# digitalcytometry/cytospace

Hardware: AMD Instinct MI355X
Metric: cell-to-spot assignments/sec on NxN synthetic cost; bit-exact vs lapjv (higher is better)
Workload: dtype f32

## Files before the change

cytospace_amd/_lib.py:

```python
import ctypes
import os

_HERE = os.path.dirname(os.path.abspath(__file__))
LIB_PATH = os.environ.get("CYTOHIP_LIB") or os.path.join(_HERE, "libcytohip.so")
_lib = None

CYTO_OK = 0
CYTO_ERR_NONFINITE = 2
_EXC = {1: ValueError, 2: ValueError, 3: MemoryError, 7: ValueError, 8: ValueError}
CYTO_ERR_PEER = 9
CYTO_ERR_UNSUPPORTED = 7
CYTO_DTYPE_F32, CYTO_DTYPE_F64, CYTO_DTYPE_U16, CYTO_DTYPE_U8, CYTO_DTYPE_I32, CYTO_DTYPE_I64 = range(6)
CYTO_MTX_ERR_FRACTION, CYTO_MTX_ERR_NONFINITE, CYTO_MTX_ERR_MAGNITUDE, CYTO_MTX_ERR_SQUARE, CYTO_MTX_ERR_IO = range(2, 7)


class CytoHipError(RuntimeError):
    pass


class LapInfo(ctypes.Structure):
    _fields_ = [("ms_colred", ctypes.c_double), ("ms_cache", ctypes.c_double), ("ms_chain", ctypes.c_double),
                ("ms_total", ctypes.c_double)] + \
        [(k, ctypes.c_int64) for k in (
            "scans_colred", "scans_redtransfer", "scans_arr", "scans_aug_init", "scans_aug_relax",
# ... 55 lines not shown
def lib():
    global _lib
    if _lib is None:
        if not os.path.exists(LIB_PATH):
            raise CytoHipError(
                f"{LIB_PATH} not found: build it with `python -m cytospace_amd.build` "
                "(hipcc --offload-arch=gfx950). There is no CPU fallback.")
        L = ctypes.CDLL(LIB_PATH)
        L.cyto_strerror.restype = ctypes.c_char_p
        L.cyto_strerror.argtypes = [ctypes.c_int]
        L.cyto_last_hip_error.restype = ctypes.c_char_p
        L.cyto_version.restype = ctypes.c_char_p
        vp, i32, i64 = ctypes.c_void_p, ctypes.c_int, ctypes.c_int64
        L.cyto_device_count.argtypes = [ctypes.POINTER(ctypes.c_int)]
        L.cyto_device_name.argtypes = [i32, ctypes.c_char_p, ctypes.c_size_t]
        L.cyto_malloc.argtypes = [ctypes.POINTER(vp), ctypes.c_size_t, i32]
        L.cyto_free.argtypes = [vp, i32]
        L.cyto_memcpy_h2d.argtypes = [vp, vp, ctypes.c_size_t, i32]
        L.cyto_memcpy_d2h.argtypes = [vp, vp, ctypes.c_size_t, i32]
        L.cyto_device_synchronize.argtypes = [i32]
        for name in ("cyto_lap_f32", "cyto_lap_f64"):
            getattr(L, name).argtypes = [i32, vp, i64, i32, vp, vp, vp, vp, ctypes.POINTER(ctypes.c_double),
                                         ctypes.POINTER(LapInfo), i32, vp]
        for name in ("cyto_lap_f32_opts", "cyto_lap_f64_opts"):
            getattr(L, name).argtypes = [i32, vp, i64, i32, vp, vp, vp, vp, ctypes.POINTER(ctypes.c_double),
                                         ctypes.POINTER(LapInfo), i32, vp, ctypes.POINTER(LapOpts)]
            getattr(L, name).restype = ctypes.c_int
        L.cyto_lap_f32_rowmap.argtypes = [i32, vp, i64, i32, i32, vp, vp, vp, vp, vp, ctypes.POINTER(ctypes.c_double),
                                          ctypes.POINTER(LapInfo), i32, vp, ctypes.POINTER(LapOpts)]
        L.cyto_lap_f32_rowmap.restype = ctypes.c_int
        if hasattr(L, "cyto_wide_embedded_solves"):
            L.cyto_wide_embedded_solves.argtypes = []
            L.cyto_wide_embedded_solves.restype = ctypes.c_longlong
        L.cyto_trim_device_cache.argtypes = [i32]
        L.cyto_trim_device_cache.restype = ctypes.c_int
        dp = ctypes.POINTER(ctypes.c_double)
        L.cyto_lap_f32_from_f64.argtypes = [i32, vp, i64, vp, vp, vp, vp, ctypes.POINTER(ctypes.c_double),
                                            ctypes.POINTER(LapInfo), i32, vp]
        L.cyto_normalize_data.argtypes = [i32, i32, vp, i64, i32, vp, i64, i32]
        L.cyto_standardize.argtypes = [i32, i32, vp, i64, i32, i32, i32, vp, i64, i32, i32, vp]
        L.cyto_cost_pearson.argtypes = [i32, i32, i32, vp, i64, vp, i64, vp, vp, i64, dp, i32, vp]
        L.cyto_transform.argtypes = [i32, i32, i32, vp, i64, i32, i32, i32, vp, i64, i32, i32, vp]
        L.cyto_cost_metric.argtypes = [i32, i32, i32, i32, vp, i64, vp, i64, vp, vp, i64, dp, i32, vp]
        L.cyto_assign_metric.argtypes = [i32, i32, i32, i32, vp, vp, vp, i32, vp, dp, ctypes.POINTER(AssignInfo), i32]
        L.cyto_assign_metric_ex.argtypes = [i32, i32, ctypes.POINTER(Matrix), i32, ctypes.POINTER(Matrix), i32, vp, i32, vp, dp,
                                            ctypes.POINTER(AssignInfo), i32]
        L.cyto_assign_metric_ex.restype = ctypes.c_int
        L.cyto_ctx_create.argtypes = [i32, i32, i32, i32, vp, vp, i32, i32, ctypes.POINTER(vp)]
        L.cyto_ctx_assign_chunk.argtypes = [vp, vp, i32, vp, i32, vp, vp, dp, ctypes.POINTER(AssignInfo)]
        L.cyto_ctx_destroy.argtypes = [vp]
        L.cyto_assign_metric_typed.argtypes = [i32, i32, i32, i32, vp, vp, i32, vp, i32, vp, dp, ctypes.POINTER(AssignInfo), i32]
        L.cyto_ctx_create_typed.argtypes = [i32, i32, i32, i32, vp, vp, i32, i32, i32, ctypes.POINTER(vp)]
        L.cyto_ctx_destroy.restype = None
        L.cyto_ctx_create_shared.argtypes = [i32, i32, i32, i32, vp, vp, i32, i32, vp, i32, i32, i32, ctypes.POINTER(vp), dp]
        L.cyto_ctx_create_shared.restype = ctypes.c_int
        L.cyto_ctx_create_ex.argtypes = [i32, i32, ctypes.POINTER(Matrix), i32, ctypes.POINTER(Matrix), i32, i32, vp, i32, i32, i32,
                                         ctypes.POINTER(vp), dp]
        L.cyto_ctx_create_ex.restype = ctypes.c_int
        L.cyto_csc_to_dense_f32.argtypes = [i32, i32, i64, vp, vp, vp, vp, i64, i32, vp]
        L.cyto_csc_to_dense_f32.restype = ctypes.c_int
        L.cyto_ctx_assign_chunks.argtypes = [vp, i32, ctypes.POINTER(Chunk), i32]
        L.cyto_ctx_assign_chunks.restype = ctypes.c_int
        L.cyto_memcpy_d2d.argtypes = [vp, vp, ctypes.c_size_t, i32]
        L.cyto_memcpy_d2d.restype = ctypes.c_int
        L.cyto_assign_pearson.argtypes = [i32, i32, i32, vp, vp, vp, i32, vp, dp, ctypes.POINTER(AssignInfo), i32]
        L.cyto_lap_batch_f32.argtypes = [i32, vp, vp, vp, i32, vp, vp, vp, vp, vp, vp, vp, i32, i32]
# ... 33 lines not shown
            getattr(L, name).restype = ctypes.c_int
        sz = [ctypes.c_size_t() for _ in range(4)]
        L.cyto_abi_sizes.argtypes = [ctypes.POINTER(ctypes.c_size_t)] * 4
        L.cyto_abi_sizes(*[ctypes.byref(x) for x in sz])
        mine = [ctypes.sizeof(t) for t in (LapInfo, LapOpts, AssignInfo, Chunk)]
        if [x.value for x in sz] != mine:
            raise CytoHipError(f"{LIB_PATH} was built from another include/cytohip.h: struct sizes {[x.value for x in sz]} != {mine} "
                               "(rebuild: python -m cytospace_amd.build --force)")
        for name in ("cyto_normalize_data", "cyto_standardize", "cyto_cost_pearson", "cyto_assign_pearson",
                     "cyto_lap_batch_f32", "cyto_lap_batch_f32_opts", "cyto_comm_unique_id", "cyto_comm_init", "cyto_comm_bcast_f32",
                     "cyto_comm_destroy"):
            getattr(L, name).restype = ctypes.c_int
        for name in ("cyto_device_count", "cyto_device_name", "cyto_malloc", "cyto_free", "cyto_memcpy_h2d",
                     "cyto_memcpy_d2h", "cyto_device_synchronize", "cyto_lap_f32", "cyto_lap_f64"):
            getattr(L, name).restype = ctypes.c_int
        _lib = L
    return _lib


def check(status):
    if status == CYTO_OK:
        return
    L = lib()
    msg = L.cyto_strerror(status).decode()
    if status == 5:
        msg += ": " + L.cyto_last_hip_error().decode()
    raise _EXC.get(status, CytoHipError)(f"cytohip status {status}: {msg}")


def wide_embedded_solves():
    return int(lib().cyto_wide_embedded_solves())


def device_count():
    n = ctypes.c_int(0)
    st = lib().cyto_device_count(ctypes.byref(n))
    return n.value if st == CYTO_OK else 0


class DeviceBuffer:

    def __init__(self, nbytes, device_id=0):
        self.device_id = device_id
        self.nbytes = int(nbytes)
        p = ctypes.c_void_p()
        check(lib().cyto_malloc(ctypes.byref(p), self.nbytes, device_id))
        self.ptr = p.value

    @classmethod
    def from_numpy(cls, arr, device_id=0):
        import numpy as np
        arr = np.ascontiguousarray(arr)
        buf = cls(arr.nbytes, device_id)
        check(lib().cyto_memcpy_h2d(buf.ptr, arr.ctypes.data, arr.nbytes, device_id))
        return buf

    def clone(self):
        out = DeviceBuffer(self.nbytes, self.device_id)
        check(lib().cyto_memcpy_d2d(out.ptr, self.ptr, self.nbytes, self.device_id))
        return out

    def to_numpy(self, shape, dtype):
        import numpy as np
        out = np.empty(shape, dtype)
        assert out.nbytes <= self.nbytes
        check(lib().cyto_memcpy_d2h(out.ctypes.data, self.ptr, out.nbytes, self.device_id))
# ... 78 lines not shown
```

cytospace_amd/csrc/lap_wide.hip:

```cpp
#include "lap_dev.h"
#include "lap_wide.h"
#include <algorithm>
#include <atomic>
#include <chrono>
#include <mutex>
#include <thread>
#include <vector>

namespace cyto {

#define WIDE_FIELDS(P, S)                                                                                                  \
    S(int, n) S(int64_t, ld) P(const float, cost) P(const int32_t, rowmap) P(float, v) P(float, u) P(float, cassign)          \
    P(unsigned long long, label) P(unsigned long long, bid) P(int32_t, rowsol) P(int32_t, colsol) P(int32_t, matches)          \
    P(int32_t, freerows) P(int32_t, act0) P(int32_t, act1) P(int32_t, touched) P(int32_t, slot_j) P(float, slot_p)            \
    P(float, slot_c) P(uint32_t, cache_col) P(float, cache_val) P(char, misc) S(long long, max_rounds)                     \
    P(const int32_t, same_prev) P(int32_t, seg_sync) S(int, aug_seg) S(int, aug_waste) S(int, arr_waste) S(int, seg_quorum)   \
    P(char, sc) S(int, par_groups) P(char, par) P(char, scx) P(float, cache_red) P(const int32_t, inv_off) P(const unsigned long long, inv_ent)
#define WIDE_F_PTR(T, name) T *name;
#define WIDE_F_VAL(T, name) T name;
struct WideArgs { WIDE_FIELDS(WIDE_F_PTR, WIDE_F_VAL) };

constexpr size_t WIDE_SC_BYTES = 2048;

namespace {

constexpr int WT = 1024;
constexpr int WNW = WT / 64;
constexpr int RTB = 256;

template <typename T> __device__ __forceinline__ T ld_sc1(const T *p) { return __hip_atomic_load(p, __ATOMIC_RELAXED, __HIP_MEMORY_SCOPE_AGENT); }
template <typename T> __device__ __forceinline__ void st_sc1(T *p, T x) { __hip_atomic_store(p, x, __ATOMIC_RELAXED, __HIP_MEMORY_SCOPE_AGENT); }
__device__ __forceinline__ int64_t wrow_off(const int32_t *__restrict__ rowmap, int i, int64_t ld) {
    return (int64_t)(rowmap ? rowmap[i] : i) * ld;
}
#define WIDE_F_GPTR(T, name) __attribute__((address_space(1))) T *name;
#define WIDE_F_COPY_PTR(T, name) a.name = (T *)g.name;
#define WIDE_F_COPY_VAL(T, name) a.name = g.name;
// ... 989 lines not shown
        h->started = 1; h->round = round; h->bids = bids; h->retired = s.retired; h->dense = s.dense; h->cnt[cur] = paused ? na : 0;
        h->cnt[cur ^ 1] = 0; h->free_cr = free_cr; h->done = paused ? 0 : 1; h->launches += 1; h->list_rounds = n_list;
#ifndef CYTO_WIDE_PROF
        tmr[WT_ARR_LAUNCHES] = h->launches;
#endif
        if (a.seg_sync) a.seg_sync[1 + blockIdx.x] = (paused ? 1 : 0) | ((!paused && s.dense <= n / 64) ? 2 : 0);
    }
}

struct ClaimCtl { int changed, blocked, rounds, pad_; };
__device__ __forceinline__ int *cl_claim(const WideArgs &a) { return reinterpret_cast<int *>(a.scx); }
__device__ __forceinline__ unsigned long long *cl_mask(const WideArgs &a) { return reinterpret_cast<unsigned long long *>(a.scx + sc_np(a.n) * 8); }
__device__ __forceinline__ int2 *cl_state(const WideArgs &a) { return reinterpret_cast<int2 *>(a.scx + sc_np(a.n) * 16); }
__device__ __forceinline__ ClaimCtl *cl_ctl(const WideArgs &a) { return reinterpret_cast<ClaimCtl *>(a.scx + sc_np(a.n) * 24); }
__device__ __forceinline__ int *cl_rem(const WideArgs &a) { return reinterpret_cast<int *>(a.scx + sc_np(a.n) * 32); }
constexpr int AP = 2;

size_t wide_aug_lds_bytes(int n, bool vlds, bool clds) {
    const size_t nblk = ((size_t)n + 63) / 64, nw32 = ((size_t)n + 31) / 32, npad = ((size_t)n + 3) & ~(size_t)3;
    return ((nblk * 8 + 3 * nw32 * 4 + npad * ((vlds ? 4 : 0) + (clds ? 2 : 0)) + 15) / 16) * 16;
}
bool wide_aug_vlds(int n) { return n <= 65534 && wide_aug_lds_bytes(n, true, true) + 4096 <= (size_t)LDS_DYNAMIC_MAX; }
bool wide_aug_clds(int n) { return n <= 65534 && wide_aug_lds_bytes(n, false, true) + 4096 <= (size_t)LDS_DYNAMIC_MAX; }

struct AugShared {
    unsigned long long T;
    int ntouch, any[3], npk[3], fail, anydense, rootdense, doroot, f, err;
    int waste, stop;
    int nhop;
    int conflict;
    int scans;
    int st_row[64], st_col[64];
    float st_val[64];
};
static_assert(WNW * 2 <= 32, "the queue of a round's full-row relaxations: two halves of the 64-entry staging arrays");

struct ParCtl {
    unsigned int bar_arrive, bar_gen;
    int P[2], nplog[2], nolog[2];
    int err, pad_;
    long long c_relax, c_hops, c_proc, c_dense, c_rounds, c_verify, c_batches, c_discarded;
};
static_assert(sizeof(ParCtl) <= 256, "control block");
constexpr int PAR_GMAX = 64;
static size_t wide_par_state_bytes(int n, int G) {
    const size_t np = ((size_t)n + 63) & ~(size_t)63;
    return 256 + (size_t)G * np * 8 + (size_t)G * np * 4 + (size_t)G * np * 8 + np * 4 + np * 8 + np * 8;
}
__device__ __forceinline__ void par_barrier(ParCtl *c, int G, unsigned &gen) {
    __syncthreads();
    if (threadIdx.x == 0) {
        __builtin_amdgcn_fence(__ATOMIC_RELEASE, "agent");
        asm volatile("s_waitcnt vmcnt(0)" ::: "memory");
        const unsigned arrived = atomicAdd(&c->bar_arrive, 1u) + 1u;
        if (arrived == (gen + 1u) * (unsigned)G) st_sc1(&c->bar_gen, gen + 1u);
        else {
            long long spins = 0;
            while (ld_sc1(&c->bar_gen) <= gen) {
                __builtin_amdgcn_s_sleep(2);
                if (++spins > (1ll << 26)) { atomicExch(&c->err, 2); break; }
            }
        }
        __builtin_amdgcn_fence(__ATOMIC_ACQUIRE, "agent");
    }
    gen++;
    __syncthreads();
}

#ifndef CYTO_COOP_MIN_N
#define CYTO_COOP_MIN_N 16384
#endif
constexpr int COOP_MIN_N = CYTO_COOP_MIN_N;
template <bool VLDS>
__device__ __forceinline__ void coop_dense_rows(AugShared *sp, int nd, const float *__restrict__ cost, const int32_t *__restrict__ rowmap, int64_t ld,
                                             int n, int w, int lane, unsigned long long *lbl, int32_t *tch, uint32_t *dirty,
                                             unsigned long long *bmin, const uint32_t *asg, const float *s_v, const float *v) {
// ... 114 lines not shown
    auto is_asg = [&](int c) -> bool { return (asg[c >> 5] >> (c & 31)) & 1u; };

    long long c_relax = 0, c_hops = 0, c_rounds = 0, c_proc = 0, c_trivial = 0, c_dense = 0, c_verify = 0;
    long long t_rounds = 0, t_verify = 0, t_finish = 0, t_triv = 0, t_mark = wall_clock64();

#define AUG_LAP(acc) { const long long now_ = wall_clock64(); acc += now_ - t_mark; t_mark = now_; }

    auto offer = [&](int col, unsigned long long lv, int row) -> unsigned long long {
        return atomicMin(lbl + col, lkey(lv, (uint32_t)row));
    };
    auto after_offer = [&](int col, unsigned long long lv, int row, unsigned long long old) {
        const unsigned long long key = lkey(lv, (uint32_t)row);
        if (key < old) {
            if (old == ~0ull) tch[atomicAdd(&s.ntouch, 1)] = col;
            if (lv_of(old) > lv) {
                const unsigned long long ck = lkey(lv, (uint32_t)col);
                if (is_asg(col)) { atomicOr(&dirty[col >> 5], 1u << (col & 31)); atomicMin(&bmin[col >> 6], ck); }
                else atomicMin(&s.T, ck);
            }
        }
    };
    auto relax_to = [&](int col, unsigned long long lv, int row) { after_offer(col, lv, row, offer(col, lv, row)); };

    int f = f0;
    int ph = 0;
    int rb[AP];
#pragma unroll
    for (int q = 0; q < AP; q++) rb[q] = -1;
    int seg_done = 0;
    int wact = 4;
    bool announced = false;
    int fbase = 0, batchno = 1, perr = 0;
    long long c_batches = 0, c_discarded = 0;
    for (;;) {
        if (!PAR && w == 0) {
            auto flush_one_edge = [&](int cnt) {
                if (lane < cnt) {
                    const int r = s.st_row[lane], cc = s.st_col[lane];
                    a.rowsol[r] = cc; a.colsol[cc] = r; a.cassign[cc] = s.st_val[lane];
                }
            };
            const int *remp = (a.same_prev && a.scx) ? cl_rem(a) : nullptr;
            int nst = 0;
            int p0, l0, r0, p1, l1, r1, p2, l2, r2, p3, l3v, r3v;
            uint32_t col0, col1, col2; float val0, val1, val2, vv0, vv1;
            auto start = [&](int ff) {
                auto len_of = [&](int pp) -> int { return pp < numfree ? (remp ? uni(remp[pp]) : 1) : 1; };
                auto row_at = [&](int pp) -> int { return pp < numfree ? uni(a.freerows[pp]) : -1; };
                p0 = ff; l0 = len_of(p0); r0 = row_at(p0);
                p1 = p0 + l0; l1 = len_of(p1); r1 = row_at(p1);
                p2 = p1 + l1; l2 = len_of(p2); r2 = row_at(p2);
                p3 = p2 + l2; l3v = p3 < numfree ? (remp ? remp[p3] : 1) : 1; r3v = p3 < numfree ? a.freerows[p3] : -1;
                col0 = COLSENT; col1 = COLSENT; col2 = COLSENT; val0 = 0.0f; val1 = 0.0f; val2 = 0.0f;
                if (r0 >= 0) { col0 = a.cache_col[(int64_t)r0 * KC + lane]; val0 = a.cache_val[(int64_t)r0 * KC + lane]; }
                if (r1 >= 0) { col1 = a.cache_col[(int64_t)r1 * KC + lane]; val1 = a.cache_val[(int64_t)r1 * KC + lane]; }
                if (r2 >= 0) { col2 = a.cache_col[(int64_t)r2 * KC + lane]; val2 = a.cache_val[(int64_t)r2 * KC + lane]; }
                vv0 = (r0 >= 0 && lane < KCU && col0 != COLSENT) ? getv((int)col0) : 0.0f;
                vv1 = (r1 >= 0 && lane < KCU && col1 != COLSENT) ? getv((int)col1) : 0.0f;
            };
            start(f);
            while (f < numfree) {
                const int fr = r0, L = l0 < 1 ? 1 : l0;
                const uint32_t col = col0;
                const float val = val0, vv = vv0;
                const int n_p3 = p3, n_l3 = uni(l3v), n_r3 = uni(r3v);
                p0 = p1; l0 = l1; r0 = r1; col0 = col1; val0 = val1; vv0 = vv1;
// ... 19 lines not shown
                    s.st_row[nst + rank] = fr + rank; s.st_col[nst + rank] = (int)col; s.st_val[nst + rank] = val;
                    if (CLDS) s_cs[col] = (uint16_t)(fr + rank);
                    atomicOr(&asg[col >> 5], 1u << (col & 31));
                }
                c_trivial += m; c_hops += m;
                f += m;
                nst += m;
                if (nst == 64) { flush_one_edge(nst); nst = 0; }
                if (m != L && f < numfree) start(f);
            }
            flush_one_edge(nst);
            if (lane == 0) {
                s.f = f;
                if (seg_done > 0 && f < numfree) {
                    bool stop = a.aug_seg > 0 && seg_done >= a.aug_seg;
                    if (a.aug_seg == 0) {
                        if (s.waste >= a.aug_waste) { stop = true; if (!announced && a.seg_sync) atomicAdd(a.seg_sync, 1); announced = true; }
                        else if (a.seg_sync && a.seg_quorum > 0 && ld_sc1(a.seg_sync) >= a.seg_quorum) stop = true;
                    }
                    if (stop) s.stop = 1;
                }
            }
        }
        __syncthreads();
        AUG_LAP(t_triv)
        if (PAR) {
            if (fbase >= numfree || perr) break;
            f = fbase + g;
        } else {
            f = uni(s.f);
            if (f >= numfree || uni(s.stop)) break;
        }
        const bool active = !PAR || f < numfree;
        seg_done++;
        const int fr = a.freerows[active ? f : 0];
        const float *__restrict__ frow = a.cost + wrow_off(a.rowmap, fr, a.ld);
        const float ftau = a.cache_val[(int64_t)fr * KC + KCU];

        if (active) {
        if (w == 0) {
            const uint32_t col = a.cache_col[(int64_t)fr * KC + lane];
            const float val = a.cache_val[(int64_t)fr * KC + lane];
            if (EMB) {
                const float red = ld_sc1(a.cache_red + (int64_t)fr * KC + lane);
                if (lane < KCU && col != COLSENT) relax_to((int)col, (unsigned long long)f2ord(red) << 12, fr);
            } else if (lane < KCU && col != COLSENT) relax_to((int)col, (unsigned long long)f2ord(val - getv((int)col)) << 12, fr);
        }
        __syncthreads();

        for (;;) {
            int nd = 0;
            for (;;) {
                const unsigned long long Tlv = uni(lv_of(s.T));
                const int W = wact;
                if (w >= W && rb[0] < 0 && rb[1] < 0) {
                    __syncthreads();
                    const int any0 = uni(s.any[ph]), npd0 = uni(s.npk[ph]), np0 = npd0 & 0xFFFF;
                    ph = (ph + 1) % 3;
                    c_rounds++;
                    wact = np0 > 6 ? WNW : 4;
                    nd = npd0 >> 16;
                    if (!any0 || nd) break;
                    continue;
                }
                unsigned long long mk = ~0ull;
                if (w < W) for (int b = w + W * lane; b < nblk; b += W * 64) mk = umin64(mk, bmin[b]);
                bool pk[AP]; int pj[AP], oi[AP];
                unsigned long long lab[AP];
                float ca[AP], vp[AP], val[AP];
                uint32_t col[AP];
                {
                    uint32_t dk = lv_of(mk) < Tlv ? (uint32_t)(mk >> 32) : 0xFFFFFFFFu;
#pragma unroll
                    for (int q = 0; q < AP; q++) {
                        const uint32_t m = wave_min_u32(dk);
                        pk[q] = m != 0xFFFFFFFFu;
                        const int l = pk[q] ? __ffsll((unsigned long long)__ballot(dk == m)) - 1 : 0;
                        pj[q] = (int)(rdlane((uint32_t)mk, l) & 0xFFFFFu);
                        if (lane == l) dk = 0xFFFFFFFFu;
                    }
                }
#pragma unroll
                for (int q = 0; q < AP; q++) {
                    if (pk[q] && lane == 0) { atomicAnd(&dirty[pj[q] >> 5], ~(1u << (pj[q] & 31))); bmin[pj[q] >> 6] = ~0ull; }
                }
                if (lane == 0 && (pk[0] || pk[1] || rb[0] >= 0 || rb[1] >= 0)) { s.any[ph] = 1; if (pk[0]) atomicAdd(&s.npk[ph], (int)pk[0] + (int)pk[1]); }
                asm volatile("s_waitcnt lgkmcnt(0)" ::: "memory");
                int pjx[AP];
                unsigned long long lab_r[AP];
                float ca_r[AP], vp_r[AP];
                int oi_r[AP];
#pragma unroll
                for (int q = 0; q < AP; q++) {
                    pjx[q] = pk[q] ? pj[q] : 0;
                    lab_r[q] = ld_sc1(lbl + pjx[q]); ca_r[q] = ld_sc1(a.cassign + pjx[q]);
                }
                bool db[AP]; unsigned long long lbr[AP];
#pragma unroll
                for (int q = 0; q < AP; q++) {
                    const int c = (rb[q] < 0 ? 0 : rb[q]) * 64 + lane;
                    db[q] = rb[q] >= 0 && c < n && ((dirty[c >> 5] >> (c & 31)) & 1u);
                    lbr[q] = ld_sc1(lbl + (db[q] ? c : pjx[q]));
                }
#pragma unroll
                for (int q = 0; q < AP; q++) { vp_r[q] = getv(pjx[q]); oi_r[q] = getcs(pjx[q]); }
#pragma unroll
                for (int q = 0; q < AP; q++) {
                    oi[q] = uni(oi_r[q]);
                    const int oix = oi[q] < 0 ? 0 : oi[q];
                    col[q] = a.cache_col[(int64_t)oix * KC + lane];
                    val[q] = EMB ? ld_sc1(a.cache_red + (int64_t)oix * KC + lane) : a.cache_val[(int64_t)oix * KC + lane];
                }
#pragma unroll
                for (int q = 0; q < AP; q++) {
                    lab[q] = pk[q] ? uni(lab_r[q]) : ~0ull; ca[q] = uni(ca_r[q]); vp[q] = uni(vp_r[q]);
                    if (!pk[q]) { col[q] = COLSENT; oi[q] = 0; }
                }
                unsigned long long old[AP], co[AP];
                bool off[AP], dn[AP];
                float vc[AP];
#pragma unroll
                for (int q = 0; q < AP; q++) {
                    const bool valid = lane < KCU && col[q] != COLSENT;
                    vc[q] = EMB ? 0.0f : getv(valid ? (int)col[q] : pjx[q]);
                }
#pragma unroll
                for (int q = 0; q < AP; q++) {
                    off[q] = false; dn[q] = false; old[q] = 0; co[q] = 0;
                    const uint32_t dord = (uint32_t)(lab[q] >> 32), kq = (uint32_t)(lab[q] >> 20) & LKMAX;
                    if (pk[q] && lv_of(lab[q]) < Tlv) {
                        c_proc++;
                        if ((dense[oi[q] >> 5] >> (oi[q] & 31)) & 1u) { dn[q] = true; continue; }
                        const float h = (ca[q] - vp[q]) - ord2f(dord);
                        const unsigned long long lv = edge_lv(f2ord(EMB ? val[q] - h : (val[q] - vc[q]) - h), dord, kq);
                        off[q] = lane < KCU && col[q] != COLSENT && (int)col[q] != pj[q] && lv <= Tlv;
                        co[q] = lv;
                    }
                }
                {
                    static_assert(AP == 2, "two offers per wave and round");
                    const uint64_t m0 = __ballot(off[0]), m1 = __ballot(off[1]);
                    if (m0 | m1) {
                        unsigned long long *p0 = lbl + (off[0] ? (int)col[0] : 0), *p1 = lbl + (off[1] ? (int)col[1] : 0);
                        const unsigned long long k0 = lkey(co[0], (uint32_t)oi[0]), k1 = lkey(co[1], (uint32_t)oi[1]);
                        unsigned long long r0, r1;
                        uint64_t sv;
                        asm volatile("s_mov_b64 %[sv], exec\n\t"
                                     "s_and_b64 exec, %[sv], %[m0]\n\t"
                                     "global_atomic_umin_x2 %[r0], %[a0], %[d0], off sc0\n\t"
                                     "s_and_b64 exec, %[sv], %[m1]\n\t"
// ... 17 lines not shown
                    const uint32_t dord = (uint32_t)(lab[q] >> 32), kq = (uint32_t)(lab[q] >> 20) & LKMAX;
                    const float h = (ca[q] - vp[q]) - ord2f(dord);
                    if (n >= COOP_MIN_N) {
                        if (lane == 0) {
                            const int e = atomicAdd(&s.npk[ph], 1 << 16) >> 16;
                            s.st_row[e] = oi[q]; s.st_row[32 + e] = pj[q]; s.st_col[e] = (int)dord; s.st_col[32 + e] = (int)kq; s.st_val[e] = h;
                        }
                    } else {
                        const float *__restrict__ row = a.cost + wrow_off(a.rowmap, oi[q], a.ld);
                        const int pjq = pj[q], oiq = oi[q];
                        wave_row_sweep(row, n, lane, [&](int c, float x) {
                            const unsigned long long lv = edge_lv(f2ord((x - getv(c)) - h), dord, kq);
                            if (c != pjq && lv <= lv_of(s.T) && (lkey(lv, (uint32_t)oiq) < ld_sc1(lbl + c))) relax_to(c, lv, oiq);
                        });
                    }
                    c_dense++;
                    if (lane == 0) atomicAdd(&s.waste, 1);
                }
#pragma unroll
                for (int q = 0; q < AP; q++) {
                    if (rb[q] >= 0) {
                        const int c = rb[q] * 64 + lane;
                        const uint32_t dk = db[q] ? (uint32_t)(lbr[q] >> 32) : 0xFFFFFFFFu;
                        const uint32_t m = wave_min_u32(dk);
                        if (m != 0xFFFFFFFFu) {
                            const int l = __ffsll((unsigned long long)__ballot(dk == m)) - 1;
                            if (lane == 0) atomicMin(&bmin[rb[q]], ((unsigned long long)m << 32) | (uint32_t)(c - lane + l));
                        }
                    }
                    rb[q] = pk[q] ? (pj[q] >> 6) : -1;
                }
                __syncthreads();
                const int any = uni(s.any[ph]), npd = uni(s.npk[ph]), np = npd & 0xFFFF;
                if (tid == 0) { s.any[(ph + 2) % 3] = 0; s.npk[(ph + 2) % 3] = 0; }
                ph = (ph + 1) % 3;
                c_rounds++;
                wact = np > 6 ? WNW : 4;
                nd = npd >> 16;
                if (!any || nd) break;
            }
            if (nd) {
                coop_dense_rows<VLDS>(&s, nd, a.cost, a.rowmap, a.ld, n, w, lane, lbl, tch, dirty, bmin, asg, s_v, a.v);
                continue;
            }
            AUG_LAP(t_rounds)
            const unsigned long long Tk = s.T;
            const uint32_t Dord = (uint32_t)(Tk >> 32);
            const float D = Tk == ~0ull ? INFINITY : ord2f(Dord);
            const int nt = s.ntouch;
            for (int q = tid; q < nt; q += WT) {
                const int k = ld_sc1(tch + q);
                const unsigned long long lbk = ld_sc1(lbl + k);
                const uint32_t dord = (uint32_t)(lbk >> 32);
                if (lv_of(lbk) < lv_of(Tk) && is_asg(k)) {
                    const int i = getcs(k);
                    if (!((dense[i >> 5] >> (i & 31)) & 1u)) {
                        const float h = (ld_sc1(a.cassign + k) - getv(k)) - ord2f(dord);
                        const float bound = a.cache_val[(int64_t)i * KC + KCU] - h;
                        if (!(bound > D)) {
                            atomicOr(&dense[i >> 5], 1u << (i & 31));
                            atomicOr(&dirty[k >> 5], 1u << (k & 31));
                            atomicMin(&bmin[k >> 6], lkey(lv_of(lbk), (uint32_t)k));
                            atomicAdd(&s.fail, 1);
                        }
                    }
                }
            }
            if (tid == 0 && !s.rootdense && !(ftau > D)) { s.rootdense = 1; s.doroot = 1; atomicAdd(&s.fail, 1); }
            c_verify++;
            __syncthreads();
            const int fail = s.fail;
            if (s.doroot)
                for (int c = tid; c < n; c += WT) {
                    const unsigned long long lv = (unsigned long long)f2ord(frow[c] - getv(c)) << 12;
                    if (lv <= lv_of(s.T) && (lkey(lv, (uint32_t)fr) < ld_sc1(lbl + c))) relax_to(c, lv, fr);
                }
            __syncthreads();
            if (tid == 0) { if (fail) s.anydense = 1; s.fail = 0; s.doroot = 0; }
            __syncthreads();
            AUG_LAP(t_verify)
            if (!fail) break;
        }

        }

        const unsigned long long Tk = active ? s.T : ~0ull;
        if (!PAR && Tk == ~0ull) { if (tid == 0) s.err = 1; __syncthreads(); break; }
        const uint32_t Dord = (uint32_t)(Tk >> 32);
        const float D = ord2f(Dord);
        const int sink = (int)lid_of(Tk);
        const int nt = active ? s.ntouch : 0;
        bool commit = true;
        int Pb = G;
        const int par = batchno & 1;
        if (PAR) {
            const bool have = Tk != ~0ull;
            if (active && !have && tid == 0) atomicExch(&pc->err, 1);
            const uint32_t key = ((uint32_t)batchno << 8) | (uint32_t)(255 - g);
            if (have) {
                for (int q = tid; q < nt; q += WT) {
                    const int k = ld_sc1(tch + q);
                    if (lv_of(ld_sc1(lbl + k)) < lv_of(Tk) && is_asg(k)) atomicMax(claim + k, key);
                }
                if (tid == 0) atomicMax(claim + sink, key);
            }
            if (tid == 0) s.conflict = 0;
            par_barrier(pc, G, pgen);
            if (have) {
                int c = 0;
                for (int q = tid; q < nt; q += WT) {
                    const int k = ld_sc1(tch + q);
                    if (lv_of(ld_sc1(lbl + k)) < lv_of(Tk) && is_asg(k) && ld_sc1(claim + k) != key) c = 1;
                }
                if (tid == 0 && ld_sc1(claim + sink) != key) c = 1;
                if (c) s.conflict = 1;
            }
            __syncthreads();
            if (tid == 0 && active && (s.conflict || !have)) atomicMin(&pc->P[par], g);
            par_barrier(pc, G, pgen);
            Pb = uni(ld_sc1(&pc->P[par]));
            Pb = Pb < G ? Pb : G;
            if (g == 0 && tid == 0) { st_sc1(&pc->P[par ^ 1], PAR_GMAX + 1); st_sc1(&pc->nplog[par ^ 1], 0); st_sc1(&pc->nolog[par ^ 1], 0); }
            commit = active && have && g < Pb;
            if (active && !commit) c_discarded++;
        }
        if (commit) {
            int myscans = 0;
            for (int q = tid; q < nt; q += WT) {
                const int k = ld_sc1(tch + q);
                const uint32_t dord = (uint32_t)(ld_sc1(lbl + k) >> 32);
                if (dord < Dord && is_asg(k)) {
                    const float vk = getv(k);
                    const float nv = (vk + ord2f(dord)) - D;
                    if (nv < vk) {
                        a.v[k] = nv; if (VLDS) s_v[k] = nv;
                        if (PAR) { const int e = atomicAdd(&pc->nplog[par], 1); plog_col[e] = k; plog_val[e] = nv; }
                    }
                    myscans++;
                }
            }
            if (myscans) atomicAdd(&s.scans, myscans);
            if (tid == 0) {
                int j = sink, nh = 0;
                for (;;) {
                    const int i = (int)lid_of(ld_sc1(lbl + j));
                    const int jn = ld_sc1(a.rowsol + i);
                    a.colsol[j] = i; a.rowsol[i] = j;
                    st_sc1(hop_i + nh, (int32_t)i); st_sc1(hop_j + nh, (int32_t)j); nh++;
                    if (CLDS) s_cs[j] = (uint16_t)i;
                    c_hops++;
                    if (i == fr) break;
                    j = jn;
                }
                s.nhop = nh;
                atomicOr(&asg[sink >> 5], 1u << (sink & 31));
            }
            __syncthreads();
            for (int q = tid; q < s.nhop; q += WT) {
                const int i = ld_sc1(hop_i + q), j = ld_sc1(hop_j + q);
                a.cassign[j] = a.cost[wrow_off(a.rowmap, i, a.ld) + j];
                if (PAR) { const int e = atomicAdd(&pc->nolog[par], 1); olog_col[e] = j; olog_own[e] = i; }
            }
        }
        for (int q = tid; q < nt; q += WT) {
            const int k = ld_sc1(tch + q);
            lbl[k] = ~0ull;
            atomicAnd(&dirty[k >> 5], ~(1u << (k & 31)));
            bmin[k >> 6] = ~0ull;
        }
        if (s.anydense) for (int q = tid; q < nw32; q += WT) dense[q] = 0;
        __syncthreads();
        if (tid == 0) { if (commit) c_relax += s.scans; s.scans = 0; s.T = ~0ull; s.ntouch = 0; s.anydense = 0; s.rootdense = 0; s.f = f + 1; }
        f++;
        __syncthreads();
        if (PAR) {
            par_barrier(pc, G, pgen);
            perr = uni(ld_sc1(&pc->err));
            const int npl = uni(ld_sc1(&pc->nplog[par])), nol = uni(ld_sc1(&pc->nolog[par]));
            if (VLDS) for (int e = tid; e < npl; e += WT) s_v[ld_sc1(plog_col + e)] = ld_sc1(plog_val + e);
            for (int e = tid; e < nol; e += WT) {
                const int col = ld_sc1(olog_col + e);
                if (CLDS) s_cs[col] = (uint16_t)ld_sc1(olog_own + e);
                atomicOr(&asg[col >> 5], 1u << (col & 31));
            }
            __syncthreads();
            const int left = numfree - fbase;
            fbase += Pb < left ? Pb : left;
            if (Pb < 1) perr = 1;
            if (EMB) {
                for (int e0 = (g * WNW + w) * 8; e0 < npl; e0 += G * WNW * 8) {
                    const bool have_e = lane < 8 && e0 + lane < npl;
                    const int k = have_e ? ld_sc1(plog_col + e0 + lane) : 0;
                    const float nv = have_e ? ld_sc1(plog_val + e0 + lane) : 0.0f;
                    embed_repair((gf32_t *)a.cache_red, (gci32_t *)a.inv_off, (gcu64_t *)a.inv_ent, __ballot(have_e), k, nv);
                }
                par_barrier(pc, G, pgen);
            }
            batchno++; c_batches++;
        }
        AUG_LAP(t_finish)
    }

    __syncthreads();
    __shared__ double s_tot[WNW];
    __shared__ long long s_wc[WNW][4];
    if (lane == 0) { s_wc[w][0] = c_proc; s_wc[w][1] = c_dense; s_wc[w][2] = c_trivial; s_wc[w][3] = (w == 0) ? c_hops : 0; }
    __syncthreads();
    long long proc = 0, dn = 0, triv = 0, hops0 = 0;
    for (int k = 0; k < WNW; k++) { proc += s_wc[k][0]; dn += s_wc[k][1]; triv += s_wc[k][2]; hops0 += s_wc[k][3]; }
    if (PAR) {
        if (tid == 0) {
            atomicAdd(reinterpret_cast<unsigned long long *>(&pc->c_relax), (unsigned long long)c_relax);
            atomicAdd(reinterpret_cast<unsigned long long *>(&pc->c_hops), (unsigned long long)hops0);
            atomicAdd(reinterpret_cast<unsigned long long *>(&pc->c_proc), (unsigned long long)proc);
            atomicAdd(reinterpret_cast<unsigned long long *>(&pc->c_dense), (unsigned long long)dn);
            atomicAdd(reinterpret_cast<unsigned long long *>(&pc->c_discarded), (unsigned long long)c_discarded);
            if (g == 0) { pc->c_rounds = c_rounds; pc->c_verify = c_verify; pc->c_batches = c_batches; }
        }
        par_barrier(pc, G, pgen);
        if (g != 0) return;
        c_relax = (long long)ld_sc1(reinterpret_cast<unsigned long long *>(&pc->c_relax));
        hops0 = (long long)ld_sc1(reinterpret_cast<unsigned long long *>(&pc->c_hops));
        proc = (long long)ld_sc1(reinterpret_cast<unsigned long long *>(&pc->c_proc));
        dn = (long long)ld_sc1(reinterpret_cast<unsigned long long *>(&pc->c_dense));
        f = perr || ld_sc1(&pc->err) ? f : numfree;
    }
    double tot = 0.0;
    for (int i = tid; i < n; i += WT) {
        const int j = ld_sc1(a.rowsol + i);
        if (j >= 0) {
            const float cij = ld_sc1(a.cassign + j);
            a.u[i] = cij - ld_sc1(a.v + j);
            tot += (double)cij;
        }
    }
#pragma unroll
    for (int off = 32; off > 0; off >>= 1) tot += __shfl_xor(tot, off);
    if (lane == 0) s_tot[w] = tot;
    __syncthreads();
    if (tid == 0) {
        double t = 0.0;
        for (int k = 0; k < WNW; k++) t += s_tot[k];
        const bool err = s.err || (PAR && (perr || ld_sc1(&pc->err)));
        LapStatus *st = lap_status(a.misc);
        st->total = t;
        long long *ctr = st->counters, *wc = st->wide;
        ctr[C_AUG_INIT] = numfree; ctr[C_AUG_RELAX] += c_relax; ctr[C_AUGS] = numfree; ctr[C_HOPS] += hops0;
        wc[WC_DENSE_AUG] += dn; wc[WC_AUG_LAUNCHES] += 1; wc[WC_AUG_ROUNDS] += c_rounds; wc[WC_AUG_PROCESSED] += proc; wc[WC_TRIVIAL] += triv; wc[WC_VERIFY_PASSES] += c_verify;
        if (err) st->status = 1;
// ... 333 lines not shown
#pragma unroll
    for (int d = 1; d < 64; d <<= 1) { const int t = __shfl_up(inc, d); if (lane >= d) inc += t; }
    __shared__ int wi[EMB_SB / 64];
    if (lane == 63) wi[w] = inc;
    __syncthreads();
    int base = 0, tot = 0, m = 0;
    for (int k = 0; k < EMB_SB / 64; k++) { base += ws[k]; tot += wt[k]; m = max(m, wm[k]); if (k < w) base += wi[k]; }
    if (j < n) off[j] = base + inc - c;
    if (blockIdx.x == 0 && tid == 0) { off[n] = tot; cnt[n] = m; }
}
__global__ __launch_bounds__(256) void embed_fill(int n, const uint32_t *__restrict__ cache_col, const float *__restrict__ cache_val,
                                                  const int32_t *__restrict__ off, const int32_t *__restrict__ rank, unsigned long long *__restrict__ ent) {
    const int lane = threadIdx.x & 63, i = blockIdx.x * 4 + (threadIdx.x >> 6);
    if (i >= n) return;
    const uint32_t col = cache_col[(int64_t)i * KC + lane];
    const float val = cache_val[(int64_t)i * KC + lane];
    if (lane < KCU && col < (uint32_t)n)
        ent[off[col] + rank[(int64_t)i * KC + lane]] = ((unsigned long long)__float_as_uint(val) << 32) | ((uint32_t)i << 6) | (uint32_t)lane;
}
static int32_t *emb_counts(const WideArgs &wa, int n) { return reinterpret_cast<int32_t *>(reinterpret_cast<char *>(wa.cache_red) + emb_off_cnt(n)); }
static int wide_build_embedded(const WideArgs &wa, int n, hipStream_t stream) {
    char *eb = reinterpret_cast<char *>(wa.cache_red);
    int32_t *cnt = emb_counts(wa, n), *bsum = reinterpret_cast<int32_t *>(eb + emb_off_bsum(n)), *rank = reinterpret_cast<int32_t *>(eb + emb_off_rank(n));
    const int nb = emb_blocks(n);
    CYTO_HIP(hipMemsetAsync(cnt, 0, ((size_t)n + 1) * 4, stream));
    hipLaunchKernelGGL(embed_red_count, dim3((n + 3) / 4), dim3(256), 0, stream, n, wa.cache_col, wa.cache_val, wa.v, wa.cache_red, cnt, rank);
    hipLaunchKernelGGL(embed_block_sums, dim3(nb), dim3(EMB_SB), 0, stream, n, cnt, bsum);
    hipLaunchKernelGGL(embed_scan, dim3(nb), dim3(EMB_SB), 0, stream, n, cnt, bsum, const_cast<int32_t *>(wa.inv_off));
    hipLaunchKernelGGL(embed_fill, dim3((n + 3) / 4), dim3(256), 0, stream, n, wa.cache_col, wa.cache_val, wa.inv_off, rank, const_cast<unsigned long long *>(wa.inv_ent));
    CYTO_HIP(hipGetLastError());
    return CYTO_OK;
}
static std::atomic<long long> g_embedded_solves{0};

static void wide_aug_lds_choice(int n, bool &vlds, bool &clds) {
    const int lds_knob = CYTO_KNOB("CYTO_AUG_LDS").set ? CYTO_KNOB("CYTO_AUG_LDS").value : 2;
    vlds = lds_knob >= 2 && wide_aug_vlds(n); clds = lds_knob >= 1 && wide_aug_clds(n);
}

static int wide_launch_aug(const WideArgs *d_args, int nb, int n, hipStream_t stream, int par_groups, bool embed) {
    bool vlds, clds;
    wide_aug_lds_choice(n, vlds, clds);
    const size_t shm = wide_aug_lds_bytes(n, vlds, clds);
    if (shm > (size_t)LDS_DYNAMIC_MAX) return CYTO_ERR_UNSUPPORTED;
    if (par_groups > 1) {
        void (*k)(const WideArgs *) = vlds ? wide_aug<true, true, true> : clds ? wide_aug<false, true, true> : wide_aug<false, false, true>;
        if (embed) {
            if (vlds) return CYTO_ERR_INTERNAL;
            k = clds ? wide_aug<false, true, true, true> : wide_aug<false, false, true, true>;
        }
        int rc = set_max_dynamic_lds(reinterpret_cast<const void *>(k));
        if (rc) return rc;
        const int pstride = CYTO_KNOB("CYTO_PAR_STRIDE").set ? std::max(1, CYTO_KNOB("CYTO_PAR_STRIDE").value) : 1;
        hipLaunchKernelGGL(k, dim3(pstride * par_groups), dim3(WT), shm, stream, d_args);
        CYTO_HIP(hipGetLastError());
        return CYTO_OK;
    }
    void (*k)(const WideArgs *) = vlds ? wide_aug<true, true, false> : clds ? wide_aug<false, true, false> : wide_aug<false, false, false>;
    int rc = set_max_dynamic_lds(reinterpret_cast<const void *>(k));
    if (rc) return rc;
    hipLaunchKernelGGL(k, dim3(nb), dim3(WT), shm, stream, d_args);
    CYTO_HIP(hipGetLastError());
    return CYTO_OK;
}

static std::atomic<int> g_par_busy[64];
// ... 48 lines not shown
            wa.cache_red = reinterpret_cast<float *>(eb);
            wa.inv_off = reinterpret_cast<int32_t *>(eb + emb_a256((size_t)n * KC * 4));
            wa.inv_ent = reinterpret_cast<unsigned long long *>(eb + emb_off_ent(n));
        }
        wa.n = n; wa.ld = j.ld; wa.cost = j.cost; wa.rowmap = j.rowmap;
        wa.v = j.fws; wa.u = j.fws + n; wa.cassign = j.fws + 3 * (int64_t)n;
        wa.label = reinterpret_cast<unsigned long long *>(j.fws + 4 * (int64_t)n);
        wa.rowsol = j.iws; wa.colsol = j.iws + n; wa.matches = j.iws + 2 * (int64_t)n; wa.freerows = j.iws + 3 * (int64_t)n;
        wa.act0 = j.iws + 4 * (int64_t)n; wa.act1 = j.iws + 5 * (int64_t)n; wa.touched = j.iws + 6 * (int64_t)n;
        wa.slot_j = j.iws + 7 * (int64_t)n;
        wa.bid = reinterpret_cast<unsigned long long *>(j.iws + 8 * (int64_t)n);
        wa.slot_p = j.state->as<float>(); wa.slot_c = wa.slot_p + n;
        wa.cache_col = j.cache_col; wa.cache_val = j.cache_val; wa.misc = j.misc;
        wa.max_rounds = pl.rounds;
        wa.aug_seg = pl.rebuild;
        wa.aug_waste = (int)std::min<long long>(1 << 30, std::max<long long>(16, (2000000ll + (long long)nl * n * n / 100) / n));
        wa.arr_waste = std::max(8, wa.aug_waste / 3);
        if (CYTO_KNOB("CYTO_ARR_WASTE").set) wa.arr_waste = std::max(1, CYTO_KNOB("CYTO_ARR_WASTE").value);
        wa.seg_quorum = nl > 1 ? std::max(1, nl / 4) : 0;
        wa.seg_sync = nullptr;
        wa.same_prev = j.same;
        wa.sc = j.state->as<char>() + sc_off;
        CYTO_HIP(hipMemsetAsync(wa.sc, 0, WIDE_SC_BYTES, stream));
        wa.scx = j.state->as<char>() + scx_off;
        CYTO_HIP(hipMemsetAsync(wa.scx, 0, wide_sc_ext_bytes(n), stream));
        CYTO_HIP(hipMemsetAsync(wa.scx, 0xFF, wide_sc_ones_bytes(n), stream));
        wa.par_groups = parg; wa.par = nullptr;
        if (parg > 0) {
            const size_t np_ = ((size_t)n + 63) & ~(size_t)63;
            wa.par = j.state->as<char>() + par_off;
            CYTO_HIP(hipMemsetAsync(wa.par, 0, 256, stream));
            const int p_init[2] = {WIDE_PAR_GMAX + 1, WIDE_PAR_GMAX + 1};
            CYTO_HIP(hipMemcpyAsync(wa.par + 8, p_init, sizeof p_init, hipMemcpyHostToDevice, stream));
            CYTO_HIP(hipMemsetAsync(wa.par + 256, 0xFF, (size_t)parg * np_ * 8, stream));
            CYTO_HIP(hipMemsetAsync(wa.par + 256 + (size_t)parg * np_ * 20, 0, np_ * 4, stream));
            CYTO_HIP(hipStreamSynchronize(stream));
        }
        CYTO_HIP(hipMemcpyAsync(wa.cassign, wa.v, nT, hipMemcpyDeviceToDevice, stream));
        CYTO_HIP(hipMemsetAsync(wa.label, 0xFF, 2 * nT, stream));
        CYTO_HIP(hipMemsetAsync(wa.bid, 0xFF, 2 * nT, stream));
    }
    DevBuf d_wa, d_sync;
    if ((rc = d_wa.alloc(sizeof(WideArgs) * nl, stream)) || (rc = d_sync.alloc(sizeof(int32_t) * ((size_t)nl + 1), stream))) return rc;
    for (WideArgs &wa : h_wa) wa.seg_sync = d_sync.as<int32_t>();
    CYTO_HIP(hipMemcpyAsync(d_wa.p, h_wa.data(), sizeof(WideArgs) * nl, hipMemcpyHostToDevice, stream));
    if ((rc = wide_launch_rt(d_wa.as<WideArgs>(), nl, n, stream))) return rc;
    std::vector<int32_t> h_sync((size_t)nl + 1, 1);
    std::vector<int32_t> caches_fresh((size_t)nl, 0);
    using BuildFn = decltype(build_caches_of);
    auto rebuild_tramp = +[](void *ctx, const int32_t *flags) -> int { return (*static_cast<BuildFn *>(ctx))(flags); };
    for (int pass = 0;; pass++) {
        if (pass && (rc = build_caches_of(h_sync.data() + 1))) return rc;
        CYTO_HIP(hipMemsetAsync(d_sync.p, 0, sizeof(int32_t), stream));
        if ((rc = wide_launch_arr(d_wa.as<WideArgs>(), nl, n, stream, pl.wipe, pass > 0, d_sync.as<int32_t>(), rebuild_tramp, &build_caches_of,
                                  nl == 1 ? &h_wa[0] : nullptr))) return rc;
        if (h_wa[0].aug_seg != 0) break;
        CYTO_HIP(hipMemcpyAsync(h_sync.data(), d_sync.p, sizeof(int32_t) * ((size_t)nl + 1), hipMemcpyDeviceToHost, stream));
        CYTO_HIP(hipStreamSynchronize(stream));
        bool done = true;
        for (int k = 0; k < nl; k++) { done = done && (h_sync[(size_t)k + 1] & 1) == 0; caches_fresh[(size_t)k] = (h_sync[(size_t)k + 1] & 2) != 0; h_sync[(size_t)k + 1] &= 1; }
        if (done) break;
    }
    const int parg = h_wa[0].par_groups;
    for (int pass = 0;; pass++) {
        if (pass == 0) {
            std::vector<int32_t> need((size_t)nl);
            for (int k = 0; k < nl; k++) need[(size_t)k] = caches_fresh[(size_t)k] ? 0 : 1;
            if ((rc = build_caches_of(need.data()))) return rc;
        } else if ((rc = build_caches_of(h_sync.data() + 1))) return rc;
        if (pass == 0) CYTO_HIP(hipEventRecord(ev_arr_done, stream));
        if (pass == 0 && parg == 0) {
            bool dup = false;
            for (int k = 0; k < nl; k++) dup = dup || h_wa[(size_t)k].same_prev != nullptr;
            if (dup && (rc = wide_launch_claims(d_wa.as<WideArgs>(), nl, n, stream, d_sync.as<int32_t>()))) return rc;
        }
        bool embed = false;
        if (parg > 0 && h_wa[0].cache_red) {
            if ((rc = wide_build_embedded(h_wa[0], n, stream))) return rc;
            embed = embed_knob >= 2;
            if (!embed) {
                int32_t longest = 0;
                CYTO_HIP(hipMemcpyAsync(&longest, emb_counts(h_wa[0], n) + n, sizeof longest, hipMemcpyDeviceToHost, stream));
                CYTO_HIP(hipStreamSynchronize(stream));
                embed = longest <= EMB_GATE;
            }
        }
        CYTO_HIP(hipMemsetAsync(d_sync.p, 0, sizeof(int32_t), stream));
        if ((rc = wide_launch_aug(d_wa.as<WideArgs>(), nl, n, stream, parg, embed))) return rc;
        if (embed) g_embedded_solves.fetch_add(1);
        if (parg > 0) { CYTO_HIP(hipStreamSynchronize(stream)); break; }
        CYTO_HIP(hipMemcpyAsync(h_sync.data(), d_sync.p, sizeof(int32_t) * ((size_t)nl + 1), hipMemcpyDeviceToHost, stream));
        CYTO_HIP(hipStreamSynchronize(stream));
        bool done = true;
        for (int k = 0; k < nl; k++) done = done && h_sync[(size_t)k + 1] == 0;
        if (done) break;
    }
    return CYTO_OK;
}

}

extern "C" long long cyto_wide_embedded_solves(void) { return cyto::g_embedded_solves.load(); }
```

include/cytohip.h:

```cpp
#ifndef CYTOHIP_H
#define CYTOHIP_H

#include <stddef.h>
#include <stdint.h>

#ifdef __cplusplus
extern "C" {
#endif

enum {
    CYTO_OK = 0,
    CYTO_ERR_BAD_ARG = 1,
    CYTO_ERR_NONFINITE = 2,
    CYTO_ERR_NOMEM = 3,
    CYTO_ERR_INTERNAL = 4,
    CYTO_ERR_HIP = 5,
    CYTO_ERR_NO_DEVICE = 6,
    CYTO_ERR_UNSUPPORTED = 7,
    CYTO_ERR_SHAPE = 8,
    CYTO_ERR_PEER = 9
};

const char *cyto_strerror(int status);
const char *cyto_last_hip_error(void);
const char *cyto_version(void);
int cyto_abi_sizes(size_t *lap_info, size_t *lap_opts, size_t *assign_info, size_t *chunk);
long long cyto_wide_embedded_solves(void);

int cyto_device_count(int *count);
int cyto_device_name(int device_id, char *buf, size_t buflen);
int cyto_malloc(void **dptr, size_t bytes, int device_id);
int cyto_free(void *dptr, int device_id);
int cyto_memcpy_h2d(void *dst, const void *src, size_t bytes, int device_id);
int cyto_memcpy_d2h(void *dst, const void *src, size_t bytes, int device_id);
int cyto_memcpy_d2d(void *dst, const void *src, size_t bytes, int device_id);
int cyto_device_synchronize(int device_id);
int cyto_trim_device_cache(int device_id);


typedef struct {
    double ms_colred;
    double ms_cache;
    double ms_chain;
    double ms_total;
    int64_t scans_colred, scans_redtransfer, scans_arr, scans_aug_init, scans_aug_relax;
    int64_t augmentations, path_hops;
    int64_t free_after_colred, free_after_arr1, free_after_arr2;
    int64_t hbm_row_reads;
    int64_t dense_refreshes;
    double ms_arr;
    double ms_aug;
    int64_t aug_scans_skipped;
    int64_t row_groups;
    int64_t aug_dense_scans;
    int64_t aug_sparse_inits;
    int64_t aug_handover;
    int64_t wide;
    int64_t wide_rounds;
    int64_t wide_retired;
    int64_t wide_dense_arr;
// ... 220 lines not shown
```

Baseline: 1.250 million.

## Cut doomed parallel augmenting searches early when a lower group claims a column

In the multi-group parallel augmentation, groups now detect claim conflicts on columns while claiming, and publish a cut index per batch. A group whose index is at or above the cut abandons its in-progress shortest-path search mid-round instead of finishing a search that would be discarded, then resets its round state. This targets wasted relaxation work on searches that lose the commit race. In exchange it adds a per-round global load of the cut word, extra atomics on claims, and a small host readback of a cut counter.

```diff
diff --git a/cytospace_amd/_lib.py b/cytospace_amd/_lib.py
--- a/cytospace_amd/_lib.py
+++ b/cytospace_amd/_lib.py
@@ -111,6 +111,9 @@
         if hasattr(L, "cyto_wide_embedded_solves"):
             L.cyto_wide_embedded_solves.argtypes = []
             L.cyto_wide_embedded_solves.restype = ctypes.c_longlong
+        if hasattr(L, "cyto_wide_cut_searches"):
+            L.cyto_wide_cut_searches.argtypes = []
+            L.cyto_wide_cut_searches.restype = ctypes.c_longlong
         L.cyto_trim_device_cache.argtypes = [i32]
         L.cyto_trim_device_cache.restype = ctypes.c_int
         dp = ctypes.POINTER(ctypes.c_double)
@@ -210,6 +213,10 @@
     return int(lib().cyto_wide_embedded_solves())
 
 
+def wide_cut_searches():
+    return int(lib().cyto_wide_cut_searches())
+
+
 def device_count():
     n = ctypes.c_int(0)
     st = lib().cyto_device_count(ctypes.byref(n))
diff --git a/cytospace_amd/csrc/lap_wide.hip b/cytospace_amd/csrc/lap_wide.hip
--- a/cytospace_amd/csrc/lap_wide.hip
+++ b/cytospace_amd/csrc/lap_wide.hip
@@ -3,6 +3,8 @@
 #include <algorithm>
 #include <atomic>
 #include <chrono>
+#include <climits>
+#include <cstddef>
 #include <mutex>
 #include <thread>
 #include <vector>
@@ -1058,6 +1060,7 @@
     int scans;
     int st_row[64], st_col[64];
     float st_val[64];
+    int cut[3];
 };
 static_assert(WNW * 2 <= 32, "the queue of a round's full-row relaxations: two halves of the 64-entry staging arrays");
 
@@ -1065,9 +1068,12 @@
     unsigned int bar_arrive, bar_gen;
     int P[2], nplog[2], nolog[2];
     int err, pad_;
-    long long c_relax, c_hops, c_proc, c_dense, c_rounds, c_verify, c_batches, c_discarded;
+    long long c_relax, c_hops, c_proc, c_dense, c_rounds, c_verify, c_batches, c_discarded, c_cut;
+    int pad2_[4];
+    int Pcut[2], cut_init, pad3_;
 };
 static_assert(sizeof(ParCtl) <= 256, "control block");
+static_assert(offsetof(ParCtl, Pcut) == 128, "the cut index: the control block's second 128-byte line");
 constexpr int PAR_GMAX = 64;
 static size_t wide_par_state_bytes(int n, int G) {
     const size_t np = ((size_t)n + 63) & ~(size_t)63;
@@ -1248,6 +1254,7 @@
     bool announced = false;
     int fbase = 0, batchno = 1, perr = 0;
     long long c_batches = 0, c_discarded = 0;
+    int c_cut = 0;
     for (;;) {
         if (!PAR && w == 0) {
             auto flush_one_edge = [&](int cnt) {
@@ -1333,7 +1340,9 @@
             if (f >= numfree || uni(s.stop)) break;
         }
         const bool active = !PAR || f < numfree;
+        bool cut = false;
         seg_done++;
+        const int par = batchno & 1;
         const int fr = a.freerows[active ? f : 0];
         const float *__restrict__ frow = a.cost + wrow_off(a.rowmap, fr, a.ld);
         const float ftau = a.cache_val[(int64_t)fr * KC + KCU];
@@ -1357,11 +1366,12 @@
                 if (w >= W && rb[0] < 0 && rb[1] < 0) {
                     __syncthreads();
                     const int any0 = uni(s.any[ph]), npd0 = uni(s.npk[ph]), np0 = npd0 & 0xFFFF;
+                    if constexpr (PAR) cut = (unsigned)uni(s.cut[ph]) <= (unsigned)g;
                     ph = (ph + 1) % 3;
                     c_rounds++;
                     wact = np0 > 6 ? WNW : 4;
                     nd = npd0 >> 16;
-                    if (!any0 || nd) break;
+                    if (!any0 || nd || cut) break;
                     continue;
                 }
                 unsigned long long mk = ~0ull;
@@ -1396,6 +1406,8 @@
                     pjx[q] = pk[q] ? pj[q] : 0;
                     lab_r[q] = ld_sc1(lbl + pjx[q]); ca_r[q] = ld_sc1(a.cassign + pjx[q]);
                 }
+                int cut_r = 0;
+                if constexpr (PAR) cut_r = ld_sc1(&pc->Pcut[par]);
                 bool db[AP]; unsigned long long lbr[AP];
 #pragma unroll
                 for (int q = 0; q < AP; q++) {
@@ -1417,6 +1429,7 @@
                     lab[q] = pk[q] ? uni(lab_r[q]) : ~0ull; ca[q] = uni(ca_r[q]); vp[q] = uni(vp_r[q]);
                     if (!pk[q]) { col[q] = COLSENT; oi[q] = 0; }
                 }
+                if constexpr (PAR) { if (w == 0 && lane == 0) s.cut[ph] = cut_r; }
                 unsigned long long old[AP], co[AP];
                 bool off[AP], dn[AP];
                 float vc[AP];
@@ -1500,13 +1513,15 @@
                 }
                 __syncthreads();
                 const int any = uni(s.any[ph]), npd = uni(s.npk[ph]), np = npd & 0xFFFF;
+                if constexpr (PAR) cut = (unsigned)uni(s.cut[ph]) <= (unsigned)g;
                 if (tid == 0) { s.any[(ph + 2) % 3] = 0; s.npk[(ph + 2) % 3] = 0; }
                 ph = (ph + 1) % 3;
                 c_rounds++;
                 wact = np > 6 ? WNW : 4;
                 nd = npd >> 16;
-                if (!any || nd) break;
-            }
+                if (!any || nd || cut) break;
+            }
+            if (PAR && cut) break;
             if (nd) {
                 coop_dense_rows<VLDS>(&s, nd, a.cost, a.rowmap, a.ld, n, w, lane, lbl, tch, dirty, bmin, asg, s_v, a.v);
                 continue;
@@ -1552,7 +1567,7 @@
 
         }
 
-        const unsigned long long Tk = active ? s.T : ~0ull;
+        const unsigned long long Tk = active && !cut ? s.T : ~0ull;
         if (!PAR && Tk == ~0ull) { if (tid == 0) s.err = 1; __syncthreads(); break; }
         const uint32_t Dord = (uint32_t)(Tk >> 32);
         const float D = ord2f(Dord);
@@ -1560,17 +1575,30 @@
         const int nt = active ? s.ntouch : 0;
         bool commit = true;
         int Pb = G;
-        const int par = batchno & 1;
         if (PAR) {
             const bool have = Tk != ~0ull;
-            if (active && !have && tid == 0) atomicExch(&pc->err, 1);
+            if (active && !have && !cut && tid == 0) atomicExch(&pc->err, 1);
+            if (cut) {
+                c_cut++;
+#pragma unroll
+                for (int q = 0; q < AP; q++) rb[q] = -1;
+                wact = 4;
+                if (tid == 0) { s.any[0] = 0; s.any[1] = 0; s.any[2] = 0; s.npk[0] = 0; s.npk[1] = 0; s.npk[2] = 0; }
+            }
             const uint32_t key = ((uint32_t)batchno << 8) | (uint32_t)(255 - g);
             if (have) {
+                auto claim_col = [&](int k) {
+                    const uint32_t old = atomicMax(claim + k, key);
+                    if ((old >> 8) == (key >> 8)) {
+                        const int go = 255 - (int)(old & 255u);
+                        if (go != g) atomicMin(&pc->Pcut[par], go < g ? g : go);
+                    }
+                };
                 for (int q = tid; q < nt; q += WT) {
                     const int k = ld_sc1(tch + q);
-                    if (lv_of(ld_sc1(lbl + k)) < lv_of(Tk) && is_asg(k)) atomicMax(claim + k, key);
-                }
-                if (tid == 0) atomicMax(claim + sink, key);
+                    if (lv_of(ld_sc1(lbl + k)) < lv_of(Tk) && is_asg(k)) claim_col(k);
+                }
+                if (tid == 0) claim_col(sink);
             }
             if (tid == 0) s.conflict = 0;
             par_barrier(pc, G, pgen);
@@ -1585,12 +1613,17 @@
             }
             __syncthreads();
             if (tid == 0 && active && (s.conflict || !have)) atomicMin(&pc->P[par], g);
+            int cut_init = 0;
+            if (g == 0 && tid == 0) cut_init = ld_sc1(&pc->cut_init);
             par_barrier(pc, G, pgen);
             Pb = uni(ld_sc1(&pc->P[par]));
             Pb = Pb < G ? Pb : G;
-            if (g == 0 && tid == 0) { st_sc1(&pc->P[par ^ 1], PAR_GMAX + 1); st_sc1(&pc->nplog[par ^ 1], 0); st_sc1(&pc->nolog[par ^ 1], 0); }
+            if (g == 0 && tid == 0) { st_sc1(&pc->P[par ^ 1], PAR_GMAX + 1); st_sc1(&pc->Pcut[par ^ 1], cut_init); st_sc1(&pc->nplog[par ^ 1], 0); st_sc1(&pc->nolog[par ^ 1], 0); }
             commit = active && have && g < Pb;
             if (active && !commit) c_discarded++;
+#ifdef CYTO_AUG_FIN_SPLIT
+            AUG_LAP(t_verify)
+#endif
         }
         if (commit) {
             int myscans = 0;
@@ -1630,6 +1663,9 @@
                 if (PAR) { const int e = atomicAdd(&pc->nolog[par], 1); olog_col[e] = j; olog_own[e] = i; }
             }
         }
+#ifdef CYTO_AUG_FIN_SPLIT
+        if (PAR) AUG_LAP(t_finish)
+#endif
         for (int q = tid; q < nt; q += WT) {
             const int k = ld_sc1(tch + q);
             lbl[k] = ~0ull;
@@ -1666,6 +1702,9 @@
             }
             batchno++; c_batches++;
         }
+#ifdef CYTO_AUG_FIN_SPLIT
+        if (PAR) AUG_LAP(t_triv) else
+#endif
         AUG_LAP(t_finish)
     }
 
@@ -1683,6 +1722,7 @@
             atomicAdd(reinterpret_cast<unsigned long long *>(&pc->c_proc), (unsigned long long)proc);
             atomicAdd(reinterpret_cast<unsigned long long *>(&pc->c_dense), (unsigned long long)dn);
             atomicAdd(reinterpret_cast<unsigned long long *>(&pc->c_discarded), (unsigned long long)c_discarded);
+            atomicAdd(reinterpret_cast<unsigned long long *>(&pc->c_cut), (unsigned long long)c_cut);
             if (g == 0) { pc->c_rounds = c_rounds; pc->c_verify = c_verify; pc->c_batches = c_batches; }
         }
         par_barrier(pc, G, pgen);
@@ -2082,6 +2122,7 @@
     return CYTO_OK;
 }
 static std::atomic<long long> g_embedded_solves{0};
+static std::atomic<long long> g_cut_searches{0};
 
 static void wide_aug_lds_choice(int n, bool &vlds, bool &clds) {
     const int lds_knob = CYTO_KNOB("CYTO_AUG_LDS").set ? CYTO_KNOB("CYTO_AUG_LDS").value : 2;
@@ -2196,6 +2237,10 @@
             CYTO_HIP(hipMemsetAsync(wa.par, 0, 256, stream));
             const int p_init[2] = {WIDE_PAR_GMAX + 1, WIDE_PAR_GMAX + 1};
             CYTO_HIP(hipMemcpyAsync(wa.par + 8, p_init, sizeof p_init, hipMemcpyHostToDevice, stream));
+            const int cut_knob = CYTO_KNOB("CYTO_AUG_CUT").set ? CYTO_KNOB("CYTO_AUG_CUT").value : 1;
+            const int cut0 = cut_knob == 0 ? INT_MIN : cut_knob < 0 ? (int)std::min(-(long long)cut_knob, (long long)WIDE_PAR_GMAX + 1) : WIDE_PAR_GMAX + 1;
+            const int cut_words[3] = {cut0, cut0, cut0};
+            CYTO_HIP(hipMemcpyAsync(wa.par + offsetof(ParCtl, Pcut), cut_words, sizeof cut_words, hipMemcpyHostToDevice, stream));
             CYTO_HIP(hipMemsetAsync(wa.par + 256, 0xFF, (size_t)parg * np_ * 8, stream));
             CYTO_HIP(hipMemsetAsync(wa.par + 256 + (size_t)parg * np_ * 20, 0, np_ * 4, stream));
             CYTO_HIP(hipStreamSynchronize(stream));
@@ -2252,7 +2297,13 @@
         CYTO_HIP(hipMemsetAsync(d_sync.p, 0, sizeof(int32_t), stream));
         if ((rc = wide_launch_aug(d_wa.as<WideArgs>(), nl, n, stream, parg, embed))) return rc;
         if (embed) g_embedded_solves.fetch_add(1);
-        if (parg > 0) { CYTO_HIP(hipStreamSynchronize(stream)); break; }
+        if (parg > 0) {
+            long long ncut = 0;
+            CYTO_HIP(hipMemcpyAsync(&ncut, h_wa[0].par + offsetof(ParCtl, c_cut), sizeof ncut, hipMemcpyDeviceToHost, stream));
+            CYTO_HIP(hipStreamSynchronize(stream));
+            g_cut_searches.fetch_add(ncut);
+            break;
+        }
         CYTO_HIP(hipMemcpyAsync(h_sync.data(), d_sync.p, sizeof(int32_t) * ((size_t)nl + 1), hipMemcpyDeviceToHost, stream));
         CYTO_HIP(hipStreamSynchronize(stream));
         bool done = true;
@@ -2265,3 +2316,4 @@
 }
 
 extern "C" long long cyto_wide_embedded_solves(void) { return cyto::g_embedded_solves.load(); }
+extern "C" long long cyto_wide_cut_searches(void) { return cyto::g_cut_searches.load(); }
diff --git a/include/cytohip.h b/include/cytohip.h
--- a/include/cytohip.h
+++ b/include/cytohip.h
@@ -26,6 +26,7 @@
 const char *cyto_version(void);
 int cyto_abi_sizes(size_t *lap_info, size_t *lap_opts, size_t *assign_info, size_t *chunk);
 long long cyto_wide_embedded_solves(void);
+long long cyto_wide_cut_searches(void);
 
 int cyto_device_count(int *count);
 int cyto_device_name(int device_id, char *buf, size_t buflen);
```

Result: no change. 1.250 million (-0.0%).
